# QZ1-boy/FCVSR

Hardware: AMD Instinct MI355X
Metric: SR frames/sec (7-frame window, 4x 180x320->720x1280) + PSNR vs ref (higher is better)
Workload: dtype bf16

## Files before the change

### fcvsr_amd/csrc/fft.hip

```cpp
#include <stdlib.h>
#include <string.h>
#include <mutex>
#include "common.h"

namespace fcvsr {

struct FftPlan {
  int N;
  int nfac;
  int fac[20];
  unsigned magic[20];
};

static bool make_plan(int N, FftPlan* p) {
  p->N = N;
  p->nfac = 0;
  int n = N;
  while (n % 8 == 0) { p->fac[p->nfac++] = 8; n /= 8; }
  while (n % 4 == 0) { p->fac[p->nfac++] = 4; n /= 4; }
  while (n % 2 == 0) { p->fac[p->nfac++] = 2; n /= 2; }
  while (n % 9 == 0) { p->fac[p->nfac++] = 9; n /= 9; }
  for (int f = 3; f <= n; f += 2) {
    while (n % f == 0) {
      if (p->nfac >= 20) return false;
// ... 572 lines not shown
  int col, chunk;
  xcd_line_chunk(&col, &chunk);
  const int b = col / Wf, kx = col - b * Wf;
  if (b >= nbatch) return;
  load_twiddles(tw, twtab, N);
  const int l = threadIdx.x & (L - 1), j = threadIdx.x >> logL;
  const int c = chunk * L + l;
  const bool live = c < n;
  const long long col0 = ((long long)b * N * Wf + kx) * ps + (live ? c : 0);
  const long long rstride = (long long)Wf * ps;
  Cx raw[R1];
  if (j < R2) {
#pragma unroll
    for (int q = 0; q < R1; ++q) {
      const float* px = in + col0 + (long long)(j + q * R2) * rstride;
      raw[q] = Cx{px[re_off], px[im_off]};
    }
  }
  for (int m = 0; m < nm; ++m) {
    if (j < R2) {
      const float* mk = masks + (long long)m * N * Wf + kx;
      float mv[R1];
#pragma unroll
      for (int q = 0; q < R1; ++q) mv[q] = mk[(j + q * R2) * Wf];
      Cx v[R1];
#pragma unroll
      for (int q = 0; q < R1; ++q) v[q] = live ? Cx{raw[q].r * mv[q], raw[q].i * mv[q]} : Cx{0.f, 0.f};
      Dft<R1, true>::run(v);
#pragma unroll
      for (int p = 0; p < R1; ++p) {
        const int idx = (j * R1 + p) * L + l;
        zr[idx] = v[p].r;
        zi[idx] = v[p].i;
      }
    }
    __syncthreads();
    if (j < R1) {
      Cx v[R2];
      stage2_load<R1, R2, true>(zr, zi, tw, j, l, L, v);
      if (live) {
        float* ob = out + (long long)m * out_band_stride + col0;
#pragma unroll
        for (int p = 0; p < R2; ++p) {
          float* px = ob + (long long)(j + p * R1) * rstride;
          px[re_off] = v[p].r;
          px[im_off] = v[p].i;
        }
      }
    }
    __syncthreads();
  }
}

template <int DT>
__device__ __forceinline__ Cx ld_pair(const float* base, long long idx) {
  if (DT == FCVSR_F32) { const float2 v = *reinterpret_cast<const float2*>(base + idx); return Cx{v.x, v.y}; }
  const unsigned v = *reinterpret_cast<const unsigned*>(reinterpret_cast<const unsigned short*>(base) + idx);
  if (DT == FCVSR_BF16) return Cx{__uint_as_float(v << 16), __uint_as_float(v & 0xffff0000u)};
  typedef __attribute__((ext_vector_type(2))) _Float16 h2;
  const h2 h = __builtin_bit_cast(h2, v);
  return Cx{(float)h[0], (float)h[1]};
}

template <int R1, int R2, int SDT>
__global__ __launch_bounds__(512, 4) void rfft_rows2_kernel(View src, int n, int H, int logL, float* spec, long long ps,
                                                         int im_off, int re_off, const float2* twtab, int nbatch) {
  constexpr int N = R1 * R2, Wf = N / 2 + 1;
  extern __shared__ __align__(16) float lds[];
  const int L = 1 << logL;
  float* zr = lds;
  float* zi = lds + N * L;
  float2* tw = reinterpret_cast<float2*>(lds + 2 * N * L);
  int grp, chunk;
  xcd_line_chunk(&grp, &chunk);
  const int row0 = grp, nrows = nbatch * H;
  if (row0 >= nrows) return;
  load_twiddles(tw, twtab, N);
  const int l = threadIdx.x & (L - 1), j = threadIdx.x >> logL;
  const int ca = chunk * 2 * L + 2 * l;
  const bool live = ca < n && j < R2;
  const int lane_off = live ? j * (int)src.sx + 2 * l : 0;
  auto issue = [&](const int row, Cx* v) {
    const int b = row / H, y = row - b * H;
    const long long sp = (long long)b * src.sb + (long long)y * src.sy + chunk * 2 * L;
#pragma unroll
    for (int q = 0; q < R1; ++q) {
      const float* bq = SDT == FCVSR_F32 ? src.p + (sp + (long long)q * R2 * src.sx)
                                         : reinterpret_cast<const float*>(reinterpret_cast<const unsigned short*>(src.p) + (sp + (long long)q * R2 * src.sx));
      const Cx ld = ld_pair<SDT>(bq, lane_off);
      v[q] = live ? ld : Cx{0.f, 0.f};
    }
  };
  {
    const int row = row0;
    if (j < R2) {
      Cx v[R1];
      issue(row, v);
      Dft<R1, false>::run(v);
#pragma unroll
      for (int p = 0; p < R1; ++p) {
        const int idx = (j * R1 + p) * L + l;
        zr[idx] = v[p].r;
        zi[idx] = v[p].i;
      }
    }
    __syncthreads();
// ... 139 lines not shown
  while (L > 1 && L / 2 >= lanes_needed) L >>= 1;
  return L;
}
static int ilog2(int v) { int r = 0; while ((1 << r) < v) ++r; return r; }

static thread_local char g_fft_path[192] = "";
struct PathLog {
  char s[sizeof(g_fft_path)];
  size_t len = 0;
  PathLog() { s[0] = 0; }
  void add(const char* pass) {
    const int w = snprintf(s + len, sizeof(s) - len, "%s%s", len ? ";" : "", pass);
    if (w > 0) len = len + (size_t)w < sizeof(s) ? len + (size_t)w : sizeof(s) - 1;
  }
  void two_stage(const char* name, const TwoStage& ts, int L) {
    char b[64];
    snprintf(b, sizeof(b), "%s<%d,%d>/L%d", name, ts.R1, ts.R2, L);
    add(b);
  }
  void plan(const char* name, int L, int vec) {
    char b[64];
    snprintf(b, sizeof(b), "%s/L%d/vec%d", name, L, vec);
    add(b);
  }
  int publish() { memcpy(g_fft_path, s, sizeof(s)); return 0; }
};

#define FCVSR_FFT2_DISPATCH(ts, CALL)                                                                        \
  do {                                                                                                       \
    switch ((ts).N) {                                                                                        \
      case 64: CALL(8, 8); break;     case 72: CALL(8, 9); break;     case 80: CALL(8, 10); break;           \
      case 96: CALL(8, 12); break;    case 128: CALL(8, 16); break;   case 144: CALL(12, 12); break;         \
      case 160: CALL(10, 16); break;  case 180: CALL(12, 15); break;  case 192: CALL(12, 16); break;         \
      case 240: CALL(15, 16); break;  case 256: CALL(16, 16); break;  case 320: CALL(16, 20); break;         \
    }                                                                                                        \
  } while (0)
#define FCVSR_FFT2_DISPATCH_COLS(ts, CALL)                                                                   \
  do {                                                                                                       \
    switch ((ts).N) {                                                                                        \
      case 64: CALL(8, 8); break;     case 72: CALL(8, 9); break;     case 80: CALL(8, 10); break;           \
      case 96: CALL(8, 12); break;    case 128: CALL(8, 16); break;   case 144: CALL(12, 12); break;         \
      case 160: CALL(10, 16); break;  case 180: CALL(12, 15); break;  case 192: CALL(12, 16); break;         \
      case 256: CALL(16, 16); break;                                                                         \
    }                                                                                                        \
  } while (0)
#define FCVSR_FFT2_DISPATCH_BANDS(ts, CALL)                                                                  \
  do {                                                                                                       \
    switch ((ts).N) {                                                                                        \
      case 64: CALL(8, 8); break;     case 72: CALL(8, 9); break;     case 80: CALL(8, 10); break;           \
      case 96: CALL(8, 12); break;    case 128: CALL(8, 16); break;   case 144: CALL(12, 12); break;         \
      case 160: CALL(10, 16); break;  case 180: CALL(12, 15); break;                                         \
    }                                                                                                        \
  } while (0)
static const TwoStage* two_stage_cols(int N) { return (N == 240 || N == 320) ? nullptr : two_stage(N); }
static const TwoStage* two_stage_bands(int N) { return (N == 192 || N == 240 || N == 256 || N == 320) ? nullptr : two_stage(N); }

static int launch_cols2(const TwoStage& ts, const float* in, float* out, long long ps, int im_off, int re_off, int n, int Wf,
                        int B, bool inverse, const float* mask, hipStream_t st, PathLog* log) {
  const float2* tw = twiddle_table(ts.N, st);
  if (!tw) return FCVSR_E_ARG;
  const int L = pick_lanes2(ts, n), logL = ilog2(L);
  const int rmax = ts.R1 > ts.R2 ? ts.R1 : ts.R2;
  const dim3 grid(cdiv(n, L), (B * Wf + 7) / 8 * 8), block((rmax * L + 63) / 64 * 64);
  const size_t lds = 8ull * ts.N * L + 8ull * ts.N;
#define FCVSR_COLS2(A_, B_)                                                                                                 \
  if (inverse && mask) hipLaunchKernelGGL((fft_cols2_kernel<A_, B_, true, true>), grid, block, lds, st, in, out, ps, im_off, \
                                          re_off, n, Wf, logL, mask, tw, B);                                                 \
  else if (inverse) hipLaunchKernelGGL((fft_cols2_kernel<A_, B_, true, false>), grid, block, lds, st, in, out, ps, im_off,   \
                                       re_off, n, Wf, logL, mask, tw, B);                                                    \
  else hipLaunchKernelGGL((fft_cols2_kernel<A_, B_, false, false>), grid, block, lds, st, in, out, ps, im_off, re_off, n,   \
                          Wf, logL, mask, tw, B)
  FCVSR_FFT2_DISPATCH_COLS(ts, FCVSR_COLS2);
#undef FCVSR_COLS2
  if (log) log->two_stage("fft_cols2", ts, L);
  return 0;
}

static int launch_cols2_bands(const TwoStage& ts, const float* in, float* out, long long out_band_stride, long long ps, int im_off,
                             int re_off, int n, int Wf, int B, const float* masks, int nm, hipStream_t st, PathLog* log) {
  const float2* tw = twiddle_table(ts.N, st);
  if (!tw) return FCVSR_E_ARG;
  const int L = pick_lanes2(ts, n), logL = ilog2(L);
  const int rmax = ts.R1 > ts.R2 ? ts.R1 : ts.R2;
  const dim3 grid(cdiv(n, L), (B * Wf + 7) / 8 * 8), block((rmax * L + 63) / 64 * 64);
  const size_t lds = 8ull * ts.N * L + 8ull * ts.N;
#define FCVSR_COLS2B(A_, B_) \
  hipLaunchKernelGGL((fft_cols2_bands_kernel<A_, B_>), grid, block, lds, st, in, out, out_band_stride, ps, im_off, re_off, n, Wf, logL, masks, nm, tw, B)
  FCVSR_FFT2_DISPATCH_BANDS(ts, FCVSR_COLS2B);
#undef FCVSR_COLS2B
  if (log) log->two_stage("fft_cols2_bands", ts, L);
  return 0;
}

static int launch_rfft_rows2(const TwoStage& ts, const fcvsr_view* src, int n, int B, int H, float* spec, long long ps, int im_off,
                             int re_off, hipStream_t st, PathLog* log) {
  const float2* tw = twiddle_table(ts.N, st);
  if (!tw) return FCVSR_E_ARG;
  const int L = pick_lanes2(ts, n / 2), logL = ilog2(L);
  const int rmax = ts.R1 > ts.R2 ? ts.R1 : ts.R2;
  const dim3 grid(cdiv(n, 2 * L), (B * H + 7) / 8 * 8), block((rmax * L + 63) / 64 * 64);
  const size_t lds = 8ull * ts.N * L + 8ull * ts.N;
#define FCVSR_ROWS2(A_, B_)                                                                                                      \
  if (src->dtype == FCVSR_F32)                                                                                                   \
    hipLaunchKernelGGL((rfft_rows2_kernel<A_, B_, FCVSR_F32>), grid, block, lds, st, to_view(*src), n, H, logL, spec, ps, im_off, \
                       re_off, tw, B);                                                                                           \
  else if (src->dtype == FCVSR_BF16)                                                                                             \
    hipLaunchKernelGGL((rfft_rows2_kernel<A_, B_, FCVSR_BF16>), grid, block, lds, st, to_view(*src), n, H, logL, spec, ps,       \
                       im_off, re_off, tw, B);                                                                                   \
  else                                                                                                                           \
    hipLaunchKernelGGL((rfft_rows2_kernel<A_, B_, FCVSR_F16>), grid, block, lds, st, to_view(*src), n, H, logL, spec, ps, im_off, \
                       re_off, tw, B)
  FCVSR_FFT2_DISPATCH(ts, FCVSR_ROWS2);
#undef FCVSR_ROWS2
  if (log) log->two_stage("rfft_rows2", ts, L);
  return 0;
}

static int launch_irfft_rows2(const TwoStage& ts, const float* spec, long long ps, int im_off, int re_off, int n, int B, int H,
                              const fcvsr_view* dst, float scale, hipStream_t st, PathLog* log) {
  const float2* tw = twiddle_table(ts.N, st);
  if (!tw) return FCVSR_E_ARG;
  const int L = pick_lanes2(ts, n / 2), logL = ilog2(L);
  const int rmax = ts.R1 > ts.R2 ? ts.R1 : ts.R2;
  const dim3 grid(cdiv(n, 2 * L), (B * H + 7) / 8 * 8), block((rmax * L + 63) / 64 * 64);
  const size_t lds = 8ull * ts.N * L + 8ull * ts.N;
#define FCVSR_IROWS2(A_, B_) \
  hipLaunchKernelGGL((irfft_rows2_kernel<A_, B_>), grid, block, lds, st, spec, ps, im_off, re_off, n, H, logL, to_view(*dst), scale, tw, B)
  FCVSR_FFT2_DISPATCH(ts, FCVSR_IROWS2);
#undef FCVSR_IROWS2
  if (log) log->two_stage("irfft_rows2", ts, L);
  return 0;
}

static bool pair_ok(const fcvsr_view* v) {
  const int al = v->dtype == FCVSR_F32 ? 8 : 4;
  return v->sc == 1 && v->sx % 2 == 0 && v->sy % 2 == 0 && v->sb % 2 == 0 && ((uintptr_t)v->ptr % al) == 0;
}

constexpr long long kFftLdsBudget = 64 * 1024;

static int pick_lanes(int N, int n_lanes_needed) {
  int L = 32;
  while (L > 1 && (16ll * N * L + 8ll * N) > kFftLdsBudget) L >>= 1;
// ... 102 lines not shown
    const int rc = launch_cols2(*tsh, spec, mid, (long long)pix_stride, im_off, re_off, n, Wf, B, true, mask, st, &log);
    if (rc) return rc;
    FCVSR_LAUNCH_CHECK();
  } else {
    const int L = pick_lanes(H, n);
    FCVSR_CHECK_ARG(16ll * H * L + 8ll * H <= 160 * 1024, "column too long for LDS");
    const size_t lds = 16ull * H * L + 8ull * H;
    (void)allow_lds(fft_cols_kernel, lds);
    dim3 grid(cdiv(n, L), (B * Wf + 7) / 8 * 8);
    const int vec = (L >= 4 && n % L == 0 && spec_ok && ((uintptr_t)mid % 16) == 0) ? 1 : 0;
    hipLaunchKernelGGL(fft_cols_kernel, grid, dim3(512), lds, st, spec, mid, (long long)pix_stride, im_off, re_off, n, H,
                       Wf, L, 1, mask, ph, vec, B);
    FCVSR_LAUNCH_CHECK();
    log.plan("fft_cols", L, vec);
  }
  const int rc = irfft_rows(mid, (long long)pix_stride, im_off, re_off, n, B, H, W, pw, spec_ok && ((uintptr_t)mid % 16) == 0, dst, st, &log);
  return rc ? rc : log.publish();
}

extern "C" int fcvsr_irfft2_bands(const float* spec, int64_t pix_stride, int im_off, int re_off, int B, int H, int W, int n,
                                  const float* masks, int n_bands, float* work, const fcvsr_view* dst, void* stream) {
  FCVSR_CHECK_ARG(spec && masks && work && dst && n_bands >= 1 && n_bands <= 16, "null argument / 1..16 bands");
  FCVSR_CHECK_ARG(B > 0 && H > 0 && W > 1 && n > 0, "bad sizes");
  const int Wf = W / 2 + 1;
  const long long band = (long long)B * H * Wf * pix_stride;
  hipStream_t st = (hipStream_t)stream;
  const TwoStage* tsh = two_stage_bands(H);
  if (!tsh) {
    for (int m = 0; m < n_bands; ++m) {
      const int rc = fcvsr_irfft2(spec, pix_stride, im_off, re_off, B, H, W, n, masks + (long long)m * H * Wf, work, &dst[m], stream);
      if (rc) return rc;
    }
    return 0;
  }
  for (int m = 0; m < n_bands; ++m)
    FCVSR_CHECK_ARG(dst[m].ptr && dst[m].dtype == FCVSR_F32 && n <= dst[m].c, "dst: f32 views with >= n channels");
  PathLog log;
  {
    const int rc = launch_cols2_bands(*tsh, spec, work, band, (long long)pix_stride, im_off, re_off, n, Wf, B, masks, n_bands, st, &log);
    if (rc) return rc;
    FCVSR_LAUNCH_CHECK();
  }
  FftPlan pw;
  FCVSR_CHECK_ARG(make_plan(W, &pw), "length has too many factors");
  for (int m = 0; m < n_bands; ++m) {
    const float* mid = work + (long long)m * band;
    const bool mid_vec = pix_stride % 4 == 0 && im_off % 4 == 0 && re_off % 4 == 0 && ((uintptr_t)mid % 16) == 0;
    const int rc = irfft_rows(mid, (long long)pix_stride, im_off, re_off, n, B, H, W, pw, mid_vec, &dst[m], st, m == 0 ? &log : nullptr);
    if (rc) return rc;
  }
  return log.publish();
}

extern "C" const char* fcvsr_last_fft_path(void) { return g_fft_path; }
```

### fcvsr_amd/engine.py

```python
from __future__ import annotations

import ctypes as C
import math
import weakref
from collections import OrderedDict
from typing import Dict, List, Optional, Tuple

import numpy as np
import torch

from . import hip
from .hip import ACT_LEAKY, ACT_NONE, ACT_PRELU, ACT_RELU, check, lib, ptr, stream_ptr, view


_MASKS: Dict[Tuple[int, int, int], torch.Tensor] = {}


def band_masks_half(Q: int, H: int, W: int) -> torch.Tensor:
    key = (Q, H, W)
    if key not in _MASKS:
        n = 1024
        step = math.sqrt((n / 2) ** 2 + (n / 2) ** 2) / Q
        d2 = (np.arange(-(n // 2), n - n // 2, 1) ** 2).astype(np.float64)
        r2 = np.power(np.sqrt(d2[:, None] + d2[None, :]), 2)
# ... 361 lines not shown
                offs = V2(view(offsets[..., 2 * i:2 * i + 2]), view(offsets[..., 2 * (A + i):2 * (A + i) + 2]))
                dv2 = V2(view(dsts[0]), view(dsts[1]))
                if fold_f1:
                    check(L.fcvsr_iac_step2_fused(prevs, offs, C.byref(k0_v), wk.data_ptr() + i * 3 * n * 64 * 2,
                                                  bk.data_ptr() + i * 3 * n * 4, fins, 0.1, B, H, W, dv2, st),
                          "fcvsr_iac_step2_fused")
                else:
                    check(L.fcvsr_iac_step2(prevs, offs, C.byref(k_v), fins, 0.1, B, H, W, dv2, st), "fcvsr_iac_step2")
                cur = dsts
        else:
            for d, fin in enumerate((x1, x3)):
                cur = fin
                fv = view(fin)
                for i in range(A):
                    g = d * A + i
                    o_v = view(offsets[..., 2 * g:2 * g + 2])
                    k_v = view(K[..., i * 3 * n:(i + 1) * 3 * n])
                    dst = al[..., d * n:(d + 1) * n] if i == A - 1 else ping[i % 2]
                    cur_v, d_v = view(cur), view(dst)
                    if fused_iac:
                        check(L.fcvsr_iac_step(C.byref(cur_v), C.byref(o_v), C.byref(k_v), C.byref(fv), 0.1, B, H, W,
                                               C.byref(d_v), st), "fcvsr_iac_step")
                    else:
                        s_v, v_v = view(s), view(vbuf)
                        check(L.fcvsr_warp(C.byref(cur_v), C.byref(o_v), B, H, W, C.byref(s_v), st), "fcvsr_warp")
                        check(L.fcvsr_sac_v(C.byref(s_v), C.byref(k_v), B, H, W, C.byref(v_v), st), "fcvsr_sac_v")
                        check(L.fcvsr_sac_h(C.byref(v_v), C.byref(k_v), C.byref(fv), 0.1, B, H, W, C.byref(d_v), st),
                              "fcvsr_sac_h")
                    cur = dst
        out = self._new(dev, B, H, W, n, dtype=fdt_act)
        self._conv("MGAA.conv3", [al], out, res=[x2])
        if self.taps is not None:
            self._tap(f"mgaa{tag}.off_f", off4[:B])
            self._tap(f"mgaa{tag}.off_b", off4[B:])
            self._tap(f"mgaa{tag}.sim", sim)
            o = offsets.permute(0, 3, 1, 2).reshape(B, 2, A, 2, H, W)
            self.taps[f"mgaa{tag}.offsets_f"] = o[:, 0].contiguous().clone()
            self.taps[f"mgaa{tag}.offsets_b"] = o[:, 1].contiguous().clone()
            self._tap(f"mgaa{tag}.al_f", al[..., :n])
            self._tap(f"mgaa{tag}.al_b", al[..., n:])
            self._tap(f"mgaa{tag}.out", out)
        return out

    def _mffr(self, x, out_dtype=torch.float32):
        m = self._model()
        n, Q = m.n_feats, m.Freq_Inv
        dev = x.device
        B, H, W, _ = x.shape
        Wf = W // 2 + 1
        L = lib()
        st = stream_ptr()
        par = self._par
        masks = self._mask(Q, H, W, dev)
        spec = self._new(dev, B, H, Wf, 2 * n)
        xv = view(x)
        check(L.fcvsr_rfft2(C.byref(xv), B, H, W, n, spec.data_ptr(), 2 * n, 0, n, st), "fcvsr_rfft2")
        bands = self._new(dev, Q, B, H, W, n)
        work = self._new(dev, Q, B, H, Wf, 2 * n)
        bvs = (hip.View * Q)(*[view(bands[q]) for q in range(Q)])
        check(L.fcvsr_irfft2_bands(spec.data_ptr(), 2 * n, 0, n, B, H, W, n, masks.data_ptr(), Q, work.data_ptr(), bvs, st),
              "fcvsr_irfft2_bands")
        freq = [bands[Q - 1 - i] for i in range(Q)]
        s_o = self._new(dev, B, H, W, n)
        nblk = (H * W + 255) // 256
        scratch = self._new(dev, 2 * B * nblk * n)
        sums = self._new(dev, 2, B, n)
        inv_hw = 1.0 / (H * W)
        mean_sum = self._channel_sum(freq[0])
        ab = [(par[f"MFFRblock.DivEnh_block.{i}.a"], par[f"MFFRblock.DivEnh_block.{i}.b"]) for i in range(Q)]
        staged = n % 4 == 0 and 256 % (n // 4) == 0 and all(f.data_ptr() % 16 == 0 for f in freq)
        s_f = self._new(dev, B, H, W, n) if (Q > 4 or not staged) else None
        check(L.fcvsr_divenh(0, 1, freq[0].data_ptr(), (s_f if s_f is not None else s_o).data_ptr(), s_o.data_ptr(),
                             ab[0][0].data_ptr(), ab[0][1].data_ptr(), mean_sum.data_ptr(), inv_hw, None, None, sums.data_ptr(),
                             scratch.data_ptr(), scratch.numel(), B, H, W, n, st), "fcvsr_divenh(reduce)")
        gates = []
        j0 = 0
        for i in range(Q):
            pre = f"MFFRblock.DivEnh_block.{i}"
            a, b = ab[i]
            first = 1 if i == 0 else 0
            g1 = self._ca_gate(sums[0], inv_hw, pre + ".ca", B, n)
            g2 = self._ca_gate(sums[1], inv_hw, pre + ".ca", B, n) if i > 0 else None
            gates.append((g1, g2))
            sums = self._new(dev, 2, B, n)
            nxt = i + 1 < Q
            if staged:
                sa = hip.DivEnhStageArgs()
                if j0 > 0:
                    sa.ck_s_f, sa.ck_s_o = s_f.data_ptr(), s_o.data_ptr()
                for k, j in enumerate(range(j0, i + 1)):
                    sa.f[k], sa.a[k], sa.b[k] = freq[j].data_ptr(), ab[j][0].data_ptr(), ab[j][1].data_ptr()
                    sa.g1[k], sa.g2[k] = gates[j][0].data_ptr(), ptr(gates[j][1])
                sa.mean_f_sum = mean_sum.data_ptr()
                if nxt:
                    sa.f_next, sa.a_next, sa.b_next = freq[i + 1].data_ptr(), ab[i + 1][0].data_ptr(), ab[i + 1][1].data_ptr()
                ckpt = nxt and i - j0 == 3
                if ckpt:
                    sa.out_s_f = s_f.data_ptr()
                if ckpt or not nxt:
                    sa.out_s_o = s_o.data_ptr()
                sa.sums, sa.scratch, sa.scratch_elems = sums.data_ptr(), scratch.data_ptr(), scratch.numel()
                sa.inv_hw, sa.n_bands, sa.B, sa.H, sa.W, sa.C = inv_hw, i - j0 + 1, B, H, W, n
                check(L.fcvsr_divenh_stage(C.byref(sa), st), "fcvsr_divenh_stage")
                if ckpt:
                    j0 = i + 1
                continue
            check(L.fcvsr_divenh_apply_next(first, freq[i].data_ptr(), s_f.data_ptr(), s_o.data_ptr(), a.data_ptr(),
                                            b.data_ptr(), mean_sum.data_ptr(), inv_hw, g1.data_ptr(), ptr(g2),
                                            freq[i + 1].data_ptr() if nxt else None,
                                            ab[i + 1][0].data_ptr() if nxt else None,
                                            ab[i + 1][1].data_ptr() if nxt else None, sums.data_ptr(),
                                            scratch.data_ptr(), scratch.numel(), B, H, W, n, st),
                  "fcvsr_divenh_apply_next")
        g = self._ca_gate(sums[0], inv_hw, "MFFRblock.ca", B, n)
# ... 390 lines not shown
```

### fcvsr_amd/hip.py

```python
from __future__ import annotations

import ctypes as C
import os
from typing import Optional, Sequence

import numpy as np
import torch

_HERE = os.path.dirname(os.path.abspath(__file__))
LIB_PATH = os.path.join(_HERE, "lib", "libfcvsr_hip.so")

F32, BF16, F16, U8, U16 = 0, 1, 2, 3, 4
ACT_NONE, ACT_RELU, ACT_LEAKY, ACT_PRELU = 0, 1, 2, 3
_DT = {torch.float32: F32, torch.bfloat16: BF16, torch.float16: F16, torch.uint8: U8, torch.uint16: U16}


class View(C.Structure):
    _fields_ = [("ptr", C.c_void_p), ("sb", C.c_int64), ("sy", C.c_int64), ("sx", C.c_int64), ("sc", C.c_int64),
                ("c", C.c_int32), ("dtype", C.c_int32)]


class GcFinishLevel(C.Structure):
    _fields_ = [("partial", C.c_void_p), ("add", C.c_void_p), ("nparts", C.c_int32)]

# ... 35 lines not shown
CROP_HFLIP, CROP_VFLIP, CROP_TRANSPOSE = 1, 2, 4


class Colour(C.Structure):
    _fields_ = [(n, C.c_int32) for n in ("shift", "chroma_loc", "y_off", "c_off", "cy", "rv", "gu", "gv", "bu", "kr", "kg", "kb",
                                         "ur", "ug", "ub", "vr", "vg", "vb")]


CHROMA_LEFT, CHROMA_CENTER = 0, 1


class ConvDesc(C.Structure):
    _fields_ = [("n_src", C.c_int32), ("src", View * 3), ("B", C.c_int32), ("H", C.c_int32), ("W", C.c_int32),
                ("kh", C.c_int32), ("kw", C.c_int32), ("stride", C.c_int32), ("pad", C.c_int32),
                ("cout", C.c_int32), ("weight", C.c_void_p), ("cout_pad", C.c_int32), ("bias", C.c_void_p),
                ("act", C.c_int32), ("slope", C.c_float), ("slope_ptr", C.c_void_p), ("n_res", C.c_int32),
                ("res", View * 2), ("res_scale", C.c_float * 2), ("dst", View), ("pixel_shuffle", C.c_int32),
                ("gc_wmask", C.c_void_p), ("gc_partial", C.c_void_p)]


PROFILE = None
COMPUTE_DTYPE = "f32"
DOMINANT_KERNEL = "conv_direct_kernel"


class HipError(RuntimeError):
    pass


_lib: Optional[C.CDLL] = None

_VP, _I, _I64, _F = C.c_void_p, C.c_int, C.c_int64, C.c_float
_PV = C.POINTER(View)
SIGNATURES = {
    "fcvsr_last_error": [],
    "fcvsr_last_conv_kernel": [],
    "fcvsr_conv2d_wgrad_scratch_elems": [C.c_int] * 7,
    "fcvsr_conv2d_wgrad": [C.c_void_p, C.c_void_p, C.c_int, C.c_int, C.c_int, C.c_int, C.c_int, C.c_int, C.c_int, C.c_void_p, C.c_void_p,
                           C.c_longlong, C.c_int, C.c_void_p],
    "fcvsr_conv2d_wgrad_mfma_eligible": [C.c_int] * 6,
    "fcvsr_conv2d_wgrad_mfma_scratch_elems": [C.c_int] * 7,
    "fcvsr_conv2d_wgrad_mfma": [C.c_void_p, C.c_void_p, C.c_int, C.c_int, C.c_int, C.c_int, C.c_int, C.c_int, C.c_int, C.c_void_p, C.c_void_p,
                                C.c_void_p, C.c_longlong, C.c_int, C.c_int, C.c_void_p],
    "fcvsr_abi_version": [],
    "fcvsr_device_count": [],
    "fcvsr_conv2d": [C.POINTER(ConvDesc), _VP],
    "fcvsr_conv2d_f32mfma": [C.POINTER(ConvDesc), _VP],
    "fcvsr_conv2d_f32mfma_eligible": [C.POINTER(ConvDesc)],
    "fcvsr_conv2d_mfma": [C.POINTER(ConvDesc), _I, _I, _VP],
    "fcvsr_conv2d_mfma_plan": [C.POINTER(ConvDesc), _I, _I, _I, _I, C.c_char_p, _I],
    "fcvsr_rfft2": [_PV, _I, _I, _I, _I, _VP, _I64, _I, _I, _VP],
    "fcvsr_irfft2": [_VP, _I64, _I, _I, _I, _I, _I, _I, _VP, _VP, _PV, _VP],
    "fcvsr_irfft2_bands": [_VP, _I64, _I, _I, _I, _I, _I, _I, _VP, _I, _VP, _PV, _VP],
    "fcvsr_last_fft_path": [],
    "fcvsr_corr_lookup": [_VP, _VP, _I64, _I, _I, _I, _I, _I, _I, _PV, _VP],
    "fcvsr_channel_sum": [_PV, _I, _I, _I, _VP, _VP, _I64, _VP],
    "fcvsr_ca_gate": [_VP, _F, _VP, _VP, _I, _I, _I, _VP, _VP],
    "fcvsr_convblk_tail": [_VP, _VP, _VP, _I, _I, _I, _I, _VP, _I64, _I, _I, _I, _I, _VP],
    "fcvsr_convblk": [_VP, _VP, _VP, _VP, _I, _VP, _VP, _VP, _I, _I, _I, _I, _VP, _VP, _I64, _VP, _I64, _I, _I, _I, _I, _VP],
    "fcvsr_convblk_heads": [_VP, _I, _VP, _VP, _VP, _VP, _VP, _VP, _I, _I, _I, _VP, _VP, _I64, _VP, _I64, _I, _I, _VP],
    "fcvsr_warp": [_PV, _PV, _I, _I, _I, _PV, _VP],
    "fcvsr_sac_v": [_PV, _PV, _I, _I, _I, _PV, _VP],
    "fcvsr_sac_h": [_PV, _PV, _PV, _F, _I, _I, _I, _PV, _VP],
    "fcvsr_iac_step": [_PV, _PV, _PV, _PV, _F, _I, _I, _I, _PV, _VP],
    "fcvsr_feat_extract": [_PV, _I, _I, _I, _VP, _VP, _I, _VP, _VP, _VP, _I, _VP],
    "fcvsr_freq_head": [_VP, _I, _I64, _I64, _VP, _VP, _VP, _VP, _VP],
    "fcvsr_convcorr_strip": [_VP, _VP, _I, _I, _I, _I, _VP, _VP, _VP, _VP, _VP],
    "fcvsr_freq_mlp3": [_VP, _VP, _I, _I64, _I64, _VP, _VP, _VP, _VP, _I64, _VP],
    "fcvsr_iac_step2": [_PV, _PV, _PV, _PV, _F, _I, _I, _I, _PV, _VP],
    "fcvsr_iac_step2_fused": [_PV, _PV, _PV, _VP, _VP, _PV, _F, _I, _I, _I, _PV, _VP],
    "fcvsr_divenh": [_I, _I, _VP, _VP, _VP, _VP, _VP, _VP, _F, _VP, _VP, _VP, _VP, _I64, _I, _I, _I, _I, _VP],
    "fcvsr_divenh_apply_next": [_I, _VP, _VP, _VP, _VP, _VP, _VP, _F, _VP, _VP, _VP, _VP, _VP, _VP, _VP, _I64, _I, _I, _I, _I, _VP],
    "fcvsr_divenh_stage": [C.POINTER(DivEnhStageArgs), _VP],
    "fcvsr_scale_add": [_VP, _VP, _VP, _I, _VP, _I, _I, _I, _I, _I, _VP],
    "fcvsr_gc_context": [_VP, _VP, _VP, _VP, _I, _I, _I, _I, _VP, _VP, _I64, _VP],
    "fcvsr_gc_finish": [_VP, _I, _VP, _VP, _I, _I, _VP, _VP],
    "fcvsr_gc_apply": [_VP, _VP, _VP, _VP, _I, _F, _I, _I, _I, _I, _VP],
    "fcvsr_xscale": [_VP, _VP, _F, _VP, _VP, _VP, _I, _I, _I, _I, _I, _VP],
    "fcvsr_gc_finish_levels": [C.POINTER(GcFinishLevel), _I, _VP, _VP, _I, _I, _VP],
    "fcvsr_gc_partial_levels": [C.POINTER(GcPartialLevel), _I, _I, _VP, _I, _VP],
    "fcvsr_gc_apply_levels": [C.POINTER(GcApplyLevel), _I, _I, _I, _F, _I, _VP],
    "fcvsr_xscale_levels": [C.POINTER(XscaleLevel), _I, _I, _I, _VP],
    "fcvsr_rcb_level0": [_VP, _VP, _VP, _VP, _VP, _VP, _VP, _F, _F, _I, _I, _I, _I, _I, _VP],
    "fcvsr_rcb_tail": [C.POINTER(RcbTailArgs), _F, _I, _I, _VP],
    "fcvsr_pixel_shuffle": [_VP, _VP, _I, _I, _I, _I, _VP],
    "fcvsr_pixel_shuffle16": [_VP, _PV, _I, _I, _I, _I, _VP],
    "fcvsr_bilinear_up4": [_PV, _I, _I, _I, _PV, _VP],
    "fcvsr_tail_fused": [_PV, _VP, _VP, _VP, _VP, _VP, _I, _I, _I, _PV, _VP],
    "fcvsr_tail_fused_base": [_PV, _VP, _VP, _VP, _VP, _VP, _PV, _I, _I, _I, _PV, _VP],
    "fcvsr_conv_last": [_PV, _VP, _VP, _I, _I, _I, _I, _PV, _VP],
    "fcvsr_pack_weight_mfma": [_VP, _I, _I, _I, _I, _VP, _I, _I, _I, _I, _VP],
    "fcvsr_pack_weights_multi_block_elems": [],
    "fcvsr_pack_weights_mfma_multi": [_VP, _I, _I, _I, _VP],
    "fcvsr_adam_multi_block_elems": [],
    "fcvsr_adam_multi": [_VP, _I, _I, _VP, _VP, _VP, _I, _F, _F, _F, _F, _F, _F, _F, _VP],
    "fcvsr_act_bwd": [_VP, _VP, _VP, _F, C.c_longlong, _VP],
    "fcvsr_colsum_scratch_elems": [C.c_longlong, _I],
    "fcvsr_colsum": [_VP, C.c_longlong, _I, _VP, _VP, C.c_longlong, _I, _VP],
    "fcvsr_iac_bwd_sac": [_VP, _VP, _VP, _VP, _PV, _F, _I, _I, _I, _I, _VP, _I, _VP, _PV, _I, _VP],
    "fcvsr_iac_bwd_warp": [_VP, _PV, _VP, _PV, _I, _I, _I, _I, _VP, _VP, _VP],
    "fcvsr_iac_bwd_warp_det_workspace": [_I, _I, _I, _I, C.POINTER(C.c_size_t)],
    "fcvsr_iac_bwd_warp_det": [_VP, _PV, _VP, _PV, _I, _I, _I, _I, _VP, _VP, _VP, C.c_size_t, _VP],
    "fcvsr_prelu_fwd": [_VP, _VP, _VP, C.c_longlong, _VP],
    "fcvsr_prelu_bwd": [_VP, _VP, _VP, _VP, _VP, _VP, C.c_longlong, _VP],
    "fcvsr_wgrad_cout1_scratch_elems": [_I, _I, _I],
    "fcvsr_wgrad_cout1": [_VP, _VP, _I, _I, _I, _I, _VP, _VP, C.c_longlong, _I, _VP],
# ... 523 lines not shown
```

### include/fcvsr_hip.h

```cpp
#ifndef FCVSR_HIP_H
#define FCVSR_HIP_H

#include <stddef.h>
#include <stdint.h>

#ifdef __cplusplus
extern "C" {
#endif

#define FCVSR_ABI_VERSION 2

enum { FCVSR_E_ARG = -1, FCVSR_E_UNSUPPORTED = -2, FCVSR_E_NOGPU = -3 };
enum { FCVSR_F32 = 0, FCVSR_BF16 = 1, FCVSR_F16 = 2 };
enum { FCVSR_U8 = 3 };
enum { FCVSR_U16 = 4 };
enum { FCVSR_ACT_NONE = 0, FCVSR_ACT_RELU = 1, FCVSR_ACT_LEAKY = 2, FCVSR_ACT_PRELU = 3 };

typedef struct fcvsr_view {
  void*   ptr;
  int64_t sb, sy, sx, sc;
  int32_t c;
  int32_t dtype;
} fcvsr_view;

// ... 42 lines not shown
int fcvsr_pack_weights_multi_block_elems(void);
int fcvsr_pack_weights_mfma_multi(const long long* tab, int n_items, int total_blocks, int dtype, void* stream);
int fcvsr_adam_multi_block_elems(void);
int fcvsr_adam_multi(const long long* tab, int n_items, int total_blocks, const float* grad, float* exp_avg, float* exp_avg_sq,
                     int t, float step_size, float bc2_sqrt, float one_minus_b1, float b2, float one_minus_b2, float eps, float wd,
                     void* stream);
int fcvsr_act_bwd(const float* g, const float* y, float* out, float slope, long long n, void* stream);
long long fcvsr_colsum_scratch_elems(long long npix, int C);
int fcvsr_colsum(const float* x, long long npix, int C, float* out, float* scratch, long long scratch_elems, int accumulate, void* stream);
int fcvsr_rcbt_nblk(int HW);
int fcvsr_rcbt_stat_elems(void);
int fcvsr_rcbt_forward(const float* r, const float* z, const float* wmask, const float* w1, const float* w2, float slope, int B, int HW,
                       int C, float* out, float* stats, float* scratch, long long scratch_elems, void* stream);
int fcvsr_rcbt_backward(const float* r, const float* g, const float* wmask, const float* w1, const float* w2, const float* stats,
                        float slope, int B, int HW, int C, float* gr, float* dwmask, float* dw1, float* dw2, float* scratch,
                        long long scratch_elems, int accumulate , void* stream);

int fcvsr_divenh_band_nblk(int HW);
int fcvsr_divenh_band_stat_elems(int C);
int fcvsr_divenh_band_forward(const float* f, const float* sf, const float* so, const float* a, const float* b, const float* w1,
                              const float* w2, int B, int HW, int C, float* sf_out, float* so_out, float* stats, float* scratch,
                              long long scratch_elems, void* stream);
int fcvsr_divenh_band_backward(const float* f, const float* sf, const float* so, const float* a, const float* b, const float* w1,
                               const float* w2, const float* stats, const float* gsf, const float* gso, int B, int HW, int C, float* gf,
                               float* gsf_out, float* gso_out, float* ga, float* gb, float* dw1, float* dw2, float* scratch,
                               long long scratch_elems, int accumulate, void* stream);
int fcvsr_corr_lookup_bwd(const float* x1f, const float* x2f, int64_t pix_stride, int B, int H, int Wf, int C, int radius, int x_count,
                          const fcvsr_view* g, float* gx1_zeroed, float* gx2_zeroed, void* stream);
int fcvsr_prelu_fwd(const float* x, const float* slope, float* y, long long n, void* stream);
int fcvsr_prelu_bwd(const float* g, const float* x, const float* slope, float* gx, float* gslope, float* scratch, long long n, void* stream);
long long fcvsr_wgrad_cout1_scratch_elems(int B, int H, int C);
int fcvsr_wgrad_cout1(const float* x, const float* gy, int B, int H, int W, int C, float* dw, float* scratch, long long scratch_elems,
                      int accumulate, void* stream);
int fcvsr_iac_bwd_sac(const float* gy, const float* yout, const float* v, const float* s, const fcvsr_view* k1, float slope, int B, int H,
                      int W, int C, float* gfin, int fin_accumulate, float* gv, const fcvsr_view* gk, int k_accumulate, void* stream);
int fcvsr_iac_bwd_warp(const float* gv, const fcvsr_view* k1, const float* prev, const fcvsr_view* off, int B, int H, int W, int C,
                       float* gprev_zeroed, float* goff, void* stream);
int fcvsr_iac_bwd_warp_det_workspace(int B, int H, int W, int C, size_t* bytes);
int fcvsr_iac_bwd_warp_det(const float* gv, const fcvsr_view* k1, const float* prev, const fcvsr_view* off, int B, int H, int W, int C,
                           float* gprev, float* goff, void* workspace, size_t workspace_bytes, void* stream);
long long fcvsr_conv2d_wgrad_mfma_groups_scratch_elems(const int* B, const int* H, const int* W, int n_groups, int cin, int cout, int kh,
                                                       int kw);
int fcvsr_conv2d_wgrad_mfma_groups(const fcvsr_view* xs, const fcvsr_view* gys, const int* B, const int* H, const int* W, int n_groups, int kh,
                                   int kw, int pad, float* dw, float* dbias, float* scratch, long long scratch_elems, int dw_accumulate,
                                   int dbias_accumulate, void* stream);
int fcvsr_up2_adjoint(const float* g, float* out, int B, int H, int W, int C, void* stream);
int fcvsr_pool2_adjoint(const float* g, float* out, int B, int H, int W, int C, void* stream);
int fcvsr_rfft2(const fcvsr_view* src, int B, int H, int W, int n,
                float* spec, int64_t pix_stride, int im_off, int re_off, void* stream);
int fcvsr_irfft2(const float* spec, int64_t pix_stride, int im_off, int re_off, int B, int H, int W, int n,
                 const float* mask, float* work, const fcvsr_view* dst, void* stream);
int fcvsr_irfft2_bands(const float* spec, int64_t pix_stride, int im_off, int re_off, int B, int H, int W, int n,
                       const float* masks, int n_bands, float* work, const fcvsr_view* dst, void* stream);
const char* fcvsr_last_fft_path(void);

int fcvsr_feat_extract(const fcvsr_view* x, int B, int H, int W, const void* w, const float* bias, int n_blk,
                       void* const* dst, const int64_t* dst_pix_stride, const int32_t* dst_ch_off, int dst_dtype,
                       void* stream);

int fcvsr_corr_lookup(const float* x1f, const float* x2f, int64_t pix_stride, int B, int H, int Wf, int C, int radius,
                      int x_count, const fcvsr_view* dst, void* stream);
int fcvsr_channel_sum(const fcvsr_view* src, int B, int H, int W, float* out, float* scratch, int64_t scratch_elems,
                      void* stream);
int fcvsr_ca_gate(const float* sum, float inv_hw, const float* w1, const float* w2, int B, int c, int cr,
                  float* gate, void* stream);
int fcvsr_convblk_tail(const float* u, const float* gate, const float* sim, int B, int ndir, int H, int Wf,
                       float* spec, int64_t pix_stride, int re_off, int im_off, int g_stride, int g0, void* stream);
int fcvsr_convblk(const float* x, const float* w1, const float* w2, const float* prelu_slope, int ksize, const float* ca_w1,
                  const float* ca_w2, const float* sim, int B, int ndir, int H, int Wf, float* u_scratch,
                  float* partial_scratch, int64_t partial_elems, float* spec, int64_t pix_stride, int re_off, int im_off,
                  int g_stride, int g0, void* stream);
int fcvsr_convblk_heads(const float* x, int n_heads, const float* const* w1, const float* const* w2,
                        const float* const* prelu_slope, const float* const* ca_w1, const float* const* ca_w2, const float* sim,
                        int B, int H, int Wf, float* u, float* partial, int64_t partial_elems, float* spec, int64_t pix_stride,
                        int re_off, int im_off, void* stream);
int fcvsr_warp(const fcvsr_view* src, const fcvsr_view* off, int B, int H, int W, const fcvsr_view* dst, void* stream);
int fcvsr_sac_v(const fcvsr_view* s, const fcvsr_view* k1, int B, int H, int W, const fcvsr_view* dst, void* stream);
int fcvsr_sac_h(const fcvsr_view* v, const fcvsr_view* k1, const fcvsr_view* feat_in, float slope,
                int B, int H, int W, const fcvsr_view* dst, void* stream);

int fcvsr_iac_step(const fcvsr_view* prev, const fcvsr_view* off, const fcvsr_view* k1, const fcvsr_view* feat_in,
                   float slope, int B, int H, int W, const fcvsr_view* dst, void* stream);
int fcvsr_iac_step2(const fcvsr_view* prev, const fcvsr_view* off, const fcvsr_view* k1, const fcvsr_view* feat_in,
                    float slope, int B, int H, int W, const fcvsr_view* dst, void* stream);
int fcvsr_iac_step2_fused(const fcvsr_view* prev, const fcvsr_view* off, const fcvsr_view* k0, const void* wk,
                          const float* kbias, const fcvsr_view* feat_in, float slope, int B, int H, int W,
                          const fcvsr_view* dst, void* stream);

int fcvsr_freq_mlp3(const float* const* xa, const float* const* xb, int n_dirs, int64_t src_pix_stride, int64_t npix,
                    const void* w0, const void* w2, const void* w4, void* const* dst, int64_t dst_pix_stride, void* stream);

int fcvsr_freq_head(const void* x, int x_dtype, int64_t x_pix_stride, int64_t npix, const void* w0, const void* w_mid,
                    const void* w_last, float* out, void* stream);
int fcvsr_convcorr_strip(const void* off, const float* corr, int B, int H, int Wf, int xs, const void* w0, const void* w_mid,
                         const void* w_last, float* off4, void* stream);

int fcvsr_divenh(int mode, int first, const float* f, float* s_f, float* s_o, const float* a, const float* b,
                 const float* mean_f_sum, float inv_hw, const float* g1, const float* g2,
                 float* sums, float* scratch, int64_t scratch_elems, int B, int H, int W, int C, void* stream);
int fcvsr_divenh_apply_next(int first, const float* f, float* s_f, float* s_o, const float* a, const float* b,
                            const float* mean_f_sum, float inv_hw, const float* g1, const float* g2,
                            const float* f_next, const float* a_next, const float* b_next, float* sums,
                            float* scratch, int64_t scratch_elems, int B, int H, int W, int C, void* stream);
typedef struct {
  const float* ck_s_f;
  const float* ck_s_o;
// ... 191 lines not shown
```

Baseline: 918.8.

## Fuse forward column FFT with banded inverse column FFTs in one kernel

Adds a fused rfft2_bands entry point in which the forward column FFT stage is done in LDS and immediately reused for every band's masked inverse column FFT. This skips writing the full forward spectrum to global memory and reading it back once per band. The engine now calls this fused path instead of separate rfft2 and irfft2_bands calls. It adds another kernel variant, and unsupported sizes fall back to the old two-call path.

```diff
diff --git a/fcvsr_amd/csrc/fft.hip b/fcvsr_amd/csrc/fft.hip
--- a/fcvsr_amd/csrc/fft.hip
+++ b/fcvsr_amd/csrc/fft.hip
@@ -648,6 +648,106 @@
   }
 }
 
+template <int R1, int R2>
+__global__ __launch_bounds__(512) void fft_cols2_fwd_bands_kernel(const float* in, float* out, long long out_band_stride, long long ps,
+                                                                  int im_off, int re_off, int n, int Wf, int logL, const float* masks,
+                                                                  int nm, const float2* twtab, int nbatch) {
+  constexpr int N = R1 * R2;
+  extern __shared__ __align__(16) float lds[];
+  const int L = 1 << logL;
+  float* zr = lds;
+  float* zi = lds + N * L;
+  float2* tw = reinterpret_cast<float2*>(lds + 2 * N * L);
+  int col, chunk;
+  xcd_line_chunk(&col, &chunk);
+  const int b = col / Wf, kx = col - b * Wf;
+  if (b >= nbatch) return;
+  load_twiddles(tw, twtab, N);
+  const int l = threadIdx.x & (L - 1), j = threadIdx.x >> logL;
+  const int c = chunk * L + l;
+  const bool live = c < n;
+  const long long col0 = ((long long)b * N * Wf + kx) * ps + (live ? c : 0);
+  const long long rstride = (long long)Wf * ps;
+  float mv[R1];
+  auto load_masks = [&](int m) {
+    const float* mk = masks + (long long)m * N * Wf + kx;
+#pragma unroll
+    for (int q = 0; q < R1; ++q) mv[q] = mk[(j + q * R2) * Wf];
+  };
+  if (j < R2) {
+    Cx v[R1];
+#pragma unroll
+    for (int q = 0; q < R1; ++q) {
+      const float* px = in + col0 + (long long)(j + q * R2) * rstride;
+      v[q] = Cx{px[re_off], px[im_off]};
+    }
+    load_masks(0);
+#pragma unroll
+    for (int q = 0; q < R1; ++q) v[q] = live ? v[q] : Cx{0.f, 0.f};
+    Dft<R1, false>::run(v);
+#pragma unroll
+    for (int p = 0; p < R1; ++p) {
+      const int idx = (j * R1 + p) * L + l;
+      zr[idx] = v[p].r;
+      zi[idx] = v[p].i;
+    }
+  }
+  __syncthreads();
+  {
+    Cx v[R2];
+    if (j < R1) stage2_load<R1, R2, false>(zr, zi, tw, j, l, L, v);
+    __syncthreads();
+    if (j < R1) {
+#pragma unroll
+      for (int p = 0; p < R2; ++p) {
+        const int idx = (j + p * R1) * L + l;
+        zr[idx] = v[p].r;
+        zi[idx] = v[p].i;
+      }
+    }
+  }
+  __syncthreads();
+  Cx raw[R1];
+  if (j < R2) {
+#pragma unroll
+    for (int q = 0; q < R1; ++q) {
+      const int idx = (j + q * R2) * L + l;
+      raw[q] = Cx{zr[idx], zi[idx]};
+    }
+  }
+  __syncthreads();
+  for (int m = 0; m < nm; ++m) {
+    if (j < R2) {
+      Cx v[R1];
+#pragma unroll
+      for (int q = 0; q < R1; ++q) v[q] = live ? Cx{raw[q].r * mv[q], raw[q].i * mv[q]} : Cx{0.f, 0.f};
+      load_masks(m + 1 < nm ? m + 1 : m);
+      Dft<R1, true>::run(v);
+#pragma unroll
+      for (int p = 0; p < R1; ++p) {
+        const int idx = (j * R1 + p) * L + l;
+        zr[idx] = v[p].r;
+        zi[idx] = v[p].i;
+      }
+    }
+    __syncthreads();
+    if (j < R1) {
+      Cx v[R2];
+      stage2_load<R1, R2, true>(zr, zi, tw, j, l, L, v);
+      if (live) {
+        float* ob = out + (long long)m * out_band_stride + col0;
+#pragma unroll
+        for (int p = 0; p < R2; ++p) {
+          float* px = ob + (long long)(j + p * R1) * rstride;
+          px[re_off] = v[p].r;
+          px[im_off] = v[p].i;
+        }
+      }
+    }
+    __syncthreads();
+  }
+}
+
 template <int DT>
 __device__ __forceinline__ Cx ld_pair(const float* base, long long idx) {
   if (DT == FCVSR_F32) { const float2 v = *reinterpret_cast<const float2*>(base + idx); return Cx{v.x, v.y}; }
@@ -893,8 +993,17 @@
       case 160: CALL(10, 16); break;  case 180: CALL(12, 15); break;                                         \
     }                                                                                                        \
   } while (0)
+#define FCVSR_FFT2_DISPATCH_FWD_BANDS(ts, CALL)                                                              \
+  do {                                                                                                       \
+    switch ((ts).N) {                                                                                        \
+      case 64: CALL(8, 8); break;     case 72: CALL(8, 9); break;     case 80: CALL(8, 10); break;           \
+      case 96: CALL(8, 12); break;    case 128: CALL(8, 16); break;   case 144: CALL(12, 12); break;         \
+      case 180: CALL(12, 15); break;                                                                         \
+    }                                                                                                        \
+  } while (0)
 static const TwoStage* two_stage_cols(int N) { return (N == 240 || N == 320) ? nullptr : two_stage(N); }
 static const TwoStage* two_stage_bands(int N) { return (N == 192 || N == 240 || N == 256 || N == 320) ? nullptr : two_stage(N); }
+static const TwoStage* two_stage_fwd_bands(int N) { return N == 160 ? nullptr : two_stage_bands(N); }
 
 static int launch_cols2(const TwoStage& ts, const float* in, float* out, long long ps, int im_off, int re_off, int n, int Wf,
                         int B, bool inverse, const float* mask, hipStream_t st, PathLog* log) {
@@ -930,6 +1039,23 @@
   FCVSR_FFT2_DISPATCH_BANDS(ts, FCVSR_COLS2B);
 #undef FCVSR_COLS2B
   if (log) log->two_stage("fft_cols2_bands", ts, L);
+  return 0;
+}
+
+static int launch_cols2_fwd_bands(const TwoStage& ts, const float* in, float* out, long long out_band_stride, long long ps,
+                                  int im_off, int re_off, int n, int Wf, int B, const float* masks, int nm, hipStream_t st,
+                                  PathLog* log) {
+  const float2* tw = twiddle_table(ts.N, st);
+  if (!tw) return FCVSR_E_ARG;
+  const int L = pick_lanes2(ts, n), logL = ilog2(L);
+  const int rmax = ts.R1 > ts.R2 ? ts.R1 : ts.R2;
+  const dim3 grid(cdiv(n, L), (B * Wf + 7) / 8 * 8), block((rmax * L + 63) / 64 * 64);
+  const size_t lds = 8ull * ts.N * L + 8ull * ts.N;
+#define FCVSR_COLS2FB(A_, B_) \
+  hipLaunchKernelGGL((fft_cols2_fwd_bands_kernel<A_, B_>), grid, block, lds, st, in, out, out_band_stride, ps, im_off, re_off, n, Wf, logL, masks, nm, tw, B)
+  FCVSR_FFT2_DISPATCH_FWD_BANDS(ts, FCVSR_COLS2FB);
+#undef FCVSR_COLS2FB
+  if (log) log->two_stage("fft_cols2_fwd_bands", ts, L);
   return 0;
 }
 
@@ -1138,4 +1264,48 @@
   return log.publish();
 }
 
+extern "C" int fcvsr_rfft2_bands(const fcvsr_view* src, int B, int H, int W, int n, int64_t pix_stride, int im_off, int re_off,
+                                 const float* masks, int n_bands, float* work, const fcvsr_view* dst, void* stream) {
+  FCVSR_CHECK_ARG(src && src->ptr && masks && work && dst && n_bands >= 1 && n_bands <= 16, "null argument / 1..16 bands");
+  FCVSR_CHECK_ARG(src->dtype == FCVSR_F32 || src->dtype == FCVSR_BF16 || src->dtype == FCVSR_F16, "bad src dtype");
+  FCVSR_CHECK_ARG(B > 0 && H > 0 && W > 1 && n > 0 && n <= src->c, "bad sizes");
+  const int Wf = W / 2 + 1;
+  const long long band = (long long)B * H * Wf * pix_stride;
+  float* spec = work + (long long)n_bands * band;
+  hipStream_t st = (hipStream_t)stream;
+  const bool spec_pair = pix_stride % 2 == 0 && im_off % 2 == 0 && re_off % 2 == 0 && ((uintptr_t)spec % 8) == 0;
+  const TwoStage* tsw = two_stage(W);
+  const TwoStage* tsh = two_stage_fwd_bands(H);
+  if (!(tsw && tsh && n % 2 == 0 && pair_ok(src) && spec_pair)) {
+    const int rc = fcvsr_rfft2(src, B, H, W, n, spec, pix_stride, im_off, re_off, stream);
+    if (rc) return rc;
+    char fwd[sizeof(g_fft_path)];
+    memcpy(fwd, g_fft_path, sizeof(fwd));
+    const int rc2 = fcvsr_irfft2_bands(spec, pix_stride, im_off, re_off, B, H, W, n, masks, n_bands, work, dst, stream);
+    if (rc2) return rc2;
+    PathLog log;
+    log.add(fwd);
+    log.add(g_fft_path);
+    return log.publish();
+  }
+  for (int m = 0; m < n_bands; ++m)
+    FCVSR_CHECK_ARG(dst[m].ptr && dst[m].dtype == FCVSR_F32 && n <= dst[m].c, "dst: f32 views with >= n channels");
+  PathLog log;
+  int rc = launch_rfft_rows2(*tsw, src, n, B, H, spec, (long long)pix_stride, im_off, re_off, st, &log);
+  if (rc) return rc;
+  FCVSR_LAUNCH_CHECK();
+  rc = launch_cols2_fwd_bands(*tsh, spec, work, band, (long long)pix_stride, im_off, re_off, n, Wf, B, masks, n_bands, st, &log);
+  if (rc) return rc;
+  FCVSR_LAUNCH_CHECK();
+  FftPlan pw;
+  FCVSR_CHECK_ARG(make_plan(W, &pw), "length has too many factors");
+  for (int m = 0; m < n_bands; ++m) {
+    const float* mid = work + (long long)m * band;
+    const bool mid_vec = pix_stride % 4 == 0 && im_off % 4 == 0 && re_off % 4 == 0 && ((uintptr_t)mid % 16) == 0;
+    rc = irfft_rows(mid, (long long)pix_stride, im_off, re_off, n, B, H, W, pw, mid_vec, &dst[m], st, m == 0 ? &log : nullptr);
+    if (rc) return rc;
+  }
+  return log.publish();
+}
+
 extern "C" const char* fcvsr_last_fft_path(void) { return g_fft_path; }
diff --git a/fcvsr_amd/engine.py b/fcvsr_amd/engine.py
--- a/fcvsr_amd/engine.py
+++ b/fcvsr_amd/engine.py
@@ -437,14 +437,12 @@
         st = stream_ptr()
         par = self._par
         masks = self._mask(Q, H, W, dev)
-        spec = self._new(dev, B, H, Wf, 2 * n)
         xv = view(x)
-        check(L.fcvsr_rfft2(C.byref(xv), B, H, W, n, spec.data_ptr(), 2 * n, 0, n, st), "fcvsr_rfft2")
         bands = self._new(dev, Q, B, H, W, n)
-        work = self._new(dev, Q, B, H, Wf, 2 * n)
+        work = self._new(dev, Q + 1, B, H, Wf, 2 * n)
         bvs = (hip.View * Q)(*[view(bands[q]) for q in range(Q)])
-        check(L.fcvsr_irfft2_bands(spec.data_ptr(), 2 * n, 0, n, B, H, W, n, masks.data_ptr(), Q, work.data_ptr(), bvs, st),
-              "fcvsr_irfft2_bands")
+        check(L.fcvsr_rfft2_bands(C.byref(xv), B, H, W, n, 2 * n, 0, n, masks.data_ptr(), Q, work.data_ptr(), bvs, st),
+              "fcvsr_rfft2_bands")
         freq = [bands[Q - 1 - i] for i in range(Q)]
         s_o = self._new(dev, B, H, W, n)
         nblk = (H * W + 255) // 256
diff --git a/fcvsr_amd/hip.py b/fcvsr_amd/hip.py
--- a/fcvsr_amd/hip.py
+++ b/fcvsr_amd/hip.py
@@ -111,6 +111,7 @@
     "fcvsr_rfft2": [_PV, _I, _I, _I, _I, _VP, _I64, _I, _I, _VP],
     "fcvsr_irfft2": [_VP, _I64, _I, _I, _I, _I, _I, _I, _VP, _VP, _PV, _VP],
     "fcvsr_irfft2_bands": [_VP, _I64, _I, _I, _I, _I, _I, _I, _VP, _I, _VP, _PV, _VP],
+    "fcvsr_rfft2_bands": [_PV, _I, _I, _I, _I, _I64, _I, _I, _VP, _I, _VP, _PV, _VP],
     "fcvsr_last_fft_path": [],
     "fcvsr_corr_lookup": [_VP, _VP, _I64, _I, _I, _I, _I, _I, _I, _PV, _VP],
     "fcvsr_channel_sum": [_PV, _I, _I, _I, _VP, _VP, _I64, _VP],
diff --git a/include/fcvsr_hip.h b/include/fcvsr_hip.h
--- a/include/fcvsr_hip.h
+++ b/include/fcvsr_hip.h
@@ -118,6 +118,8 @@
                  const float* mask, float* work, const fcvsr_view* dst, void* stream);
 int fcvsr_irfft2_bands(const float* spec, int64_t pix_stride, int im_off, int re_off, int B, int H, int W, int n,
                        const float* masks, int n_bands, float* work, const fcvsr_view* dst, void* stream);
+int fcvsr_rfft2_bands(const fcvsr_view* src, int B, int H, int W, int n, int64_t pix_stride, int im_off, int re_off,
+                      const float* masks, int n_bands, float* work, const fcvsr_view* dst, void* stream);
 const char* fcvsr_last_fft_path(void);
 
 int fcvsr_feat_extract(const fcvsr_view* x, int B, int H, int W, const void* w, const float* bias, int n_blk,
```

Result: no change. 916.4 (-0.3%).
